# jimsnow/glome

Hardware: AMD Instinct MI355X
Metric: Mrays/sec + fps at 1920x1080 primary+shadow; 1/2/4/8 MI355X (higher is better)
Workload: dtype f32; 1 GPU; S3: 100,352-triangle heightfield under bih (BASELINE configs[2]), 1 light, primary + shadow rays, maxdepth 1; width=1920, height=1080, sampling=renderTile, 1 primary ray/pixel, launches_in_flight=4, frames_per_launch=32, transport=none (one GPU), frame_product=packed 0x00RRGGBB framebuffer (trace + blitTile fused, 4 B/pixel), bih_build=device (glome_sb_bih_dev / glome_sb_mesh_dev) for lists of 4096+ objects, device_bytes=14337692

## Files before the change

glome_amd/csrc/cull_kernels.hpp:

```cpp
#pragma once
#include <hip/hip_runtime.h>

#include "kernel_launch.hpp"
#include "rt_device.hpp"
#include "tiles.hpp"

constexpr int kCullThreads = 1024;
constexpr int kCullWaves = kCullThreads / 64, kCullPerWave = (int)kQueueChunk / kCullWaves;
static_assert(kCullWaves * kCullPerWave == (int)kQueueChunk && kQueueChunk == 64, "a chunk's live mask is one 64-bit word, a lane per position");

__device__ __forceinline__ bool queue_position(const DRenderArgs& A, uint32_t w, uint32_t& frame, uint32_t& item) {
  if (A.chunks_per_frame) {
    const uint32_t g = w / kQueueChunk, nf = (uint32_t)A.nframes;
    if (g >= A.chunks_per_frame * nf) return false;
    const uint32_t q = g / nf;
    frame = g - q * nf;
    w = q * kQueueChunk + (w % kQueueChunk);
    if (w >= A.total_waves) return false;
  } else {
    if (w >= A.total_waves * (uint32_t)A.nframes) return false;
    frame = w / A.total_waves;
    w -= frame * A.total_waves;
  }
  item = w;
  return true;
}

__device__ __forceinline__ bool item_live(const DScene& S, const Ray& r, bool valid) {
  for (uint32_t e = 0; e < S.n_entries; e++) {
    U4 ent = ldu4(S.entries, e);
    ent.x = uni(ent.x); ent.z = uni(ent.z);
    if (ent.z & RF_NOVIS) continue;
    U4 rec = ldu4(S.recs, ent.x);
    rec.x = uni(rec.x); rec.y = uni(rec.y);
    if ((rec.x & RF_KINDMASK) != R_BIH) return true;
    const F4 h0 = ld4u(S.bihhdr, 3 * rec.y), h1 = ld4u(S.bihhdr, 3 * rec.y + 1);
    if (uni(as_u(h0.w)) & BREF_LEAF) return true;
    float nearv, farv;
    bih_root_interval(r, h0, h1, kInf, nearv, farv);
    bih_clip_root_at_origin(nearv);
    if (wave_ballot(bih_root_enters(valid, nearv, farv)) != 0) return true;
  }
  return false;
}

__global__ void __launch_bounds__(kCullThreads) k_cull_items(DRenderArgs, uint32_t* list, uint32_t* masks, uint32_t nchunks) {
  const DRenderArgs& A = kernel_args<DRenderArgs>();
  __shared__ uint32_t s_bits[2], s_last, s_wave[kCullWaves], s_lo[kCullThreads], s_hi[kCullThreads], s_off[kCullThreads];
  const uint32_t tid = threadIdx.x, lane = tid & 63u, wave = tid >> 6, g = blockIdx.x;
  if (tid < 2) s_bits[tid] = 0;
  __syncthreads();
  uint32_t dead_px = 0;
  for (uint32_t k = 0; k < (uint32_t)kCullPerWave; k++) {
    const uint32_t j = wave * kCullPerWave + k;
    uint32_t frame, item;
    if (!queue_position(A, g * kQueueChunk + j, frame, item)) continue;
    const DItem it = ld_item_u(A.items, item);
    int px = 0, py = 0;
    size_t dense_off = 0;
    const bool valid = item_pixel(it, A.tiles, (int)lane, px, py, dense_off);
    const float xc = ldf(A.xc_tab, valid ? (uint32_t)px : 0u), yc = ldf(A.yc_tab, valid ? (uint32_t)py : 0u);
    const Ray ray = primary_ray(frame == 0 ? A.cam : A.more_cams[frame - 1], xc, yc);
    if (item_live(A.S, ray, valid)) {
      if (lane == 0) atomicOr(&s_bits[j >> 5], 1u << (j & 31u));
    } else {
      dead_px += (uint32_t)__builtin_popcountll(wave_ballot(valid));
      float depth = kInf;
      asm volatile("" : "+v"(depth));
      if (valid) store_pixel(A, frame, px, py, dense_off, ca(0, 0, 0, 0), depth);
    }
  }
  if (A.want_counters && dead_px && lane == 0) atomicAdd(&A.counters->rays_primary, (unsigned long long)dead_px);
  __syncthreads();
  if (tid == 0) {
    __hip_atomic_store(&masks[2 * g], s_bits[0], __ATOMIC_RELAXED, __HIP_MEMORY_SCOPE_AGENT);
    __hip_atomic_store(&masks[2 * g + 1], s_bits[1], __ATOMIC_RELAXED, __HIP_MEMORY_SCOPE_AGENT);
    asm volatile("s_waitcnt vmcnt(0)" ::: "memory");
    s_last = atomicAdd(&A.counters->cull_done, 1u) == nchunks - 1u ? 1u : 0u;
  }
  __syncthreads();
  if (!s_last) return;

  uint32_t running = 0;
  for (uint32_t base = 0; base < nchunks; base += kCullThreads) {
    const uint32_t c = base + tid;
    uint32_t lo = 0, hi = 0;
    if (c < nchunks) {
      lo = __hip_atomic_load(&masks[2 * c], __ATOMIC_RELAXED, __HIP_MEMORY_SCOPE_AGENT);
      hi = __hip_atomic_load(&masks[2 * c + 1], __ATOMIC_RELAXED, __HIP_MEMORY_SCOPE_AGENT);
    }
    const uint32_t cnt = (uint32_t)__builtin_popcount(lo) + (uint32_t)__builtin_popcount(hi);
    uint32_t incl = cnt;
    for (int o = 1; o < 64; o <<= 1) { const uint32_t v = __shfl_up(incl, o, 64); if ((int)lane >= o) incl += v; }
    if (lane == 63) s_wave[wave] = incl;
    __syncthreads();
    uint32_t before = 0, total = 0;
    for (uint32_t w = 0; w < (uint32_t)kCullWaves; w++) { const uint32_t v = s_wave[w]; total += v; if (w < wave) before += v; }
    s_lo[tid] = lo; s_hi[tid] = hi; s_off[tid] = running + before + incl - cnt;
    __syncthreads();
    for (uint32_t k = 0; k < 64; k++) {
      const uint32_t i = wave * 64 + k, ck = base + i;
      if (ck >= nchunks) break;
      const unsigned long long m = (unsigned long long)s_lo[i] | ((unsigned long long)s_hi[i] << 32);
      if (m == 0) continue;
      if ((m >> lane) & 1ull) {
        uint32_t frame = 0, item = 0;
        (void)queue_position(A, ck * kQueueChunk + lane, frame, item);
        list[s_off[i] + (uint32_t)__builtin_popcountll(m & ((1ull << lane) - 1ull))] = (frame << kListFrameShift) | item;
      }
    }
    running += total;
    __syncthreads();
  }
  if (tid == 0) {
    __hip_atomic_store(&A.counters->list_len, running, __ATOMIC_RELAXED, __HIP_MEMORY_SCOPE_AGENT);
    __hip_atomic_store(&A.counters->cull_done, 0u, __ATOMIC_RELAXED, __HIP_MEMORY_SCOPE_AGENT);
  }
}
```

glome_amd/csrc/runtime.hip:

```cpp
#include <hip/hip_runtime.h>

#include <cmath>
#include <cstdio>
#include <cstring>
#include <map>
#include <set>
#include <mutex>
#include <string>
#include <type_traits>
#include <vector>

#include "../../include/glome_hip.h"
#include "capi_shared.hpp"
#include "flatten.hpp"
#include "tiles.hpp"
#include "rt_device.hpp"
#include "instances.hpp"
#include "kernel_launch.hpp"
#include "bih_build_device.hpp"
#include "cull_kernels.hpp"
#include "mesh_update_kernels.hpp"
#include "bih_update_kernels.hpp"
#include "item_bih_update_kernels.hpp"
#include "sphere_bih_update_kernels.hpp"
// ... 422 lines not shown
    for (auto& b : boxes) bb = box_join(bb, b);
    if (bb.lo.x == -kInfinity || bb.lo.y == -kInfinity || bb.lo.z == -kInfinity || bb.hi.x == kInfinity || bb.hi.y == kInfinity || bb.hi.z == kInfinity)
      throw scene_error("bih: infinite bounding box");
    HIPCHK(ctx, hipSetDevice(ctx->device));
    auto T = std::make_shared<BihTree>();
    std::string err;
    if (!bihdev::build(boxes, v, bb, *T, ctx->stream, err, gpu_ms)) { ctx->err = sb->err = err; return GLOME_E_LIMIT; }
    T->order = v;
    Node nd; nd.kind = K_BIH; nd.bih = T;
    return G.add(nd);
  } catch (const scene_error& e) { ctx->err = sb->err = e.what(); return GLOME_E_SCENE; }
  catch (const std::exception& e) { ctx->err = sb->err = e.what(); return GLOME_E_INVALID; }
}

int32_t glome_sb_mesh_dev(glome_ctx* ctx, glome_sb* sb, const double* verts, int nv, const double* norms, int nn, const int32_t* tris, int nt, const int32_t* mats, int nm,
                          float* gpu_ms) {
  if (!ctx || !sb) { g_global_error = "null ctx or builder"; return GLOME_E_INVALID; }
  if (gpu_ms) *gpu_ms = 0;
  try {
    if (nv < 0 || nn < 0 || nt < 0 || nm < 0 || (nv && !verts) || (nn && !norms) || (nt && !tris) || (nm && !mats)) throw std::invalid_argument("bad mesh arrays");
    Graph& G = sb->graph;
    std::vector<D3> V, N;
    for (int k = 0; k < nv; k++) V.push_back(D3{verts[3 * k], verts[3 * k + 1], verts[3 * k + 2]});
    for (int k = 0; k < nn; k++) N.push_back(D3{norms[3 * k], norms[3 * k + 1], norms[3 * k + 2]});
    std::vector<MeshTri> T;
    for (int k = 0; k < nt; k++) { const int32_t* t = tris + 8 * k; T.push_back(MeshTri{t[0], t[1], t[2], t[3], t[4], t[5], t[6], t[7]}); }
    std::vector<int> M(mats, mats + nm);
    if (nt < 3) return G.mesh(std::move(V), std::move(N), std::move(T), std::move(M));
    std::vector<Box3> tbb;
    auto D = G.mesh_data(std::move(V), std::move(N), std::move(T), std::move(M), tbb);
    HIPCHK(ctx, hipSetDevice(ctx->device));
    std::string err;
    if (!bihdev::build_mesh(tbb, *D, ctx->stream, err, gpu_ms)) { ctx->err = sb->err = err; return GLOME_E_LIMIT; }
    return G.mesh_node(D);
  } catch (const scene_error& e) { ctx->err = sb->err = e.what(); return GLOME_E_SCENE; }
  catch (const std::exception& e) { ctx->err = sb->err = e.what(); return GLOME_E_INVALID; }
}

glome_scene* glome_scene_commit(glome_ctx* ctx, glome_sb* sb, int32_t root) {
  if (!ctx || !sb) { g_global_error = "null ctx or builder"; return nullptr; }
  FlatScene F;
  try {
    Flattener fl(sb_graph(sb), F);
    fl.run(root);
  } catch (std::exception& e) { ctx->err = e.what(); return nullptr; }
  (void)hipSetDevice(ctx->device);
  glome_scene* s = new glome_scene();
  s->ctx = ctx;
  int rc = 0;
  DScene& D = s->dev;
  rc |= upload(s, F.recs, &D.recs);
  rc |= upload(s, F.spheres, &D.spheres); rc |= upload(s, F.tris, &D.tris); rc |= upload(s, F.tripairs, &D.tripairs); rc |= upload(s, F.trinorms, &D.trinorms);
  rc |= upload(s, F.boxes, &D.boxes); rc |= upload(s, F.planes, &D.planes); rc |= upload(s, F.discs, &D.discs);
  rc |= upload(s, F.quadrics, &D.quadrics); rc |= upload(s, F.xfms, &D.xfms);
  rc |= upload(s, F.bihhdr, &D.bihhdr); rc |= upload(s, F.bihnodes, &D.bihnodes); rc |= upload(s, F.pknodes, &D.pknodes); D.pknodes_bytes = (uint32_t)(F.pknodes.size() * sizeof(F4));
  rc |= upload(s, F.meshhdr, &D.meshhdr); rc |= upload(s, F.meshnodes, &D.meshnodes); rc |= upload(s, F.mtris, &D.mtris);
  rc |= upload(s, F.mtrimeta, &D.mtrimeta); rc |= upload(s, F.mats, &D.mats); rc |= upload(s, F.wlights, &D.wlights); rc |= upload(s, F.matkids, &D.matkids);
  rc |= upload(s, F.entries, &D.entries);
  if (rc) { glome_scene_release(s); return nullptr; }
  D.n_entries = F.tier == 0 ? (uint32_t)F.entries.size() : 0;
  D.root_rec = F.root_rec; D.tier = F.tier; D.n_mats = (uint32_t)sb_graph(sb).mats.size(); D.tex_bits = F.tex_bits;
  const CommitRules R = commit_rules(sb_graph(sb), F);
  D.pk_generic_cap = R.caps.pk_generic_cap;
  if (getenv("GLOME_DEBUG_NO_GENERIC_PACKETS")) D.pk_generic_cap = 0;
  glome_scene_info& I = s->info;
  I.tier = (int32_t)F.tier; I.nesting_depth = F.nesting_depth;
  I.n_records = (int64_t)F.recs.size(); I.n_bih_nodes = (int64_t)F.bihnodes.size(); I.n_mesh_nodes = (int64_t)F.meshnodes.size() / 4;
  I.n_triangles = (int64_t)(F.tris.size() + F.mtris.size()) / 3; I.n_spheres = (int64_t)F.spheres.size();
  I.n_other_prims = F.n_other_prims; I.n_xfms = (int64_t)F.xfms.size() / 6; I.n_materials = D.n_mats;
  I.max_bih_depth = F.max_bih_depth; I.max_mesh_depth = F.max_mesh_depth;
  s->tr = R.traits;
  s->ovf_cap = R.caps.ovf_cap;
  for (MeshUpdateInfo& U : F.mesh_updates) {
    glome_scene::MeshUpd& m = s->meshes[U.node];
    if (upload(s, U.rows, &m.d_rows) || (!U.level_nodes.empty() && upload(s, U.level_nodes, &m.d_levels))) { glome_scene_release(s); return nullptr; }
    U.rows = {}; U.level_nodes = {};
    m.info = std::move(U);
  }
  for (LeafBihUpdateInfo& U : F.leaf_bih_updates) {
    glome_scene::LeafBihUpd& m = s->leaf_bihs[U.node];
    if ((!U.rows.empty() && upload(s, U.rows, &m.d_rows)) || (!U.level_nodes.empty() && (upload(s, U.level_nodes, &m.d_levels) || upload(s, U.level_off, &m.d_level_off)))) { glome_scene_release(s); return nullptr; }
    U.rows = {}; U.level_nodes = {};
    m.info = std::move(U);
  }
  for (InstBihInfo& B : F.inst_bihs) {
    glome_scene::InstBih& m = s->ibihs[B.node];
    if ((!B.level_nodes.empty() && upload(s, B.level_nodes, &m.d_levels)) || upload(s, B.rec_off, &m.d_rec_off) || upload(s, B.child_bound, &m.d_bounds)) { glome_scene_release(s); return nullptr; }
    B.level_nodes = {};
    m.info = std::move(B);
  }
  for (InstanceUpdateInfo& U : F.inst_updates) { const int node = U.node; s->insts[node] = std::move(U); }
  auto live_row = [&](int node, const double* b6) { s->live_slot[node] = (uint32_t)(s->live_bound0.size() / 6); s->live_bound0.insert(s->live_bound0.end(), b6, b6 + 6); };
  for (auto& m : s->meshes) live_row(m.first, m.second.info.bound6);
  for (auto& m : s->leaf_bihs) live_row(m.first, m.second.info.bound6);
  for (auto& m : s->ibihs) live_row(m.first, m.second.info.bound6);
  return s;
}
void glome_scene_release(glome_scene* s) {
  if (!s) return;
  (void)hipSetDevice(s->ctx->device);
  for (void* p : s->allocs) (void)hipFree(p);
  for (auto& st : s->inst_stage) { if (st.h) (void)hipHostFree(st.h); if (st.ev) (void)hipEventDestroy(st.ev); }
  if (s->d_inst_rows) (void)hipFree(s->d_inst_rows);
  delete s;
}
int glome_scene_get_info(const glome_scene* s, glome_scene_info* out) {
  if (!s || !out) return GLOME_E_INVALID;
  *out = s->info;
  return 0;
}

static bool other_slots_busy(glome_ctx* ctx) {
  for (int k = 0; k < glome_ctx::kSlots; k++) {
    const glome_ctx::Slot& sl = ctx->slots[k];
    if (k == ctx->cur || !sl.launched_on || sl.launched_on == ctx->stream) continue;
    if (hipStreamQuery(sl.launched_on) == hipErrorNotReady) return true;
  }
  (void)hipGetLastError();
  return false;
}
static int persistent_grid(glome_ctx* ctx, size_t lds_per_block, uint32_t total_work, int max_per_cu = 32, int min_per_cu = 0) {
  int cus = ctx->prop.multiProcessorCount;
  int per_cu = max_per_cu;
  if (lds_per_block) per_cu = std::min<int>(per_cu, (int)(160 * 1024 / lds_per_block));
  per_cu = std::max(per_cu, 1);
  if (ctx->grid_per_cu > 0) per_cu = std::min(per_cu, ctx->grid_per_cu);
  else if (min_per_cu > 0) {
    const bool alone = !other_slots_busy(ctx);
    const long per_wave = alone ? 16L : 64L;
    if (alone && min_per_cu >= 8) min_per_cu = 12;
    long want = ((long)total_work + per_wave * cus - 1) / (per_wave * cus);
    per_cu = (int)std::min<long>(per_cu, std::max<long>(min_per_cu, want));
  }
  long g = (long)cus * per_cu;
  return (int)std::max<long>(1, std::min<long>(g, total_work));
}
static int grid_floor(const glome_scene* s) { return s->tr.n_bih_nodes + s->tr.n_mesh_nodes < 4096 ? 3 : 8; }
static int ensure_overflow(glome_ctx* ctx, int grid, int waves_per_block, int ovf_cap) {
  size_t need = (size_t)grid * waves_per_block * (ovf_cap + 1) * 3 * 64 * sizeof(uint32_t);
  glome_ctx::Slot& sl = ctx->slot();
  if (need <= sl.ovf_bytes) return 0;
  if (sl.d_ovf) { HIPCHK(ctx, hipStreamSynchronize(ctx->stream)); HIPCHK(ctx, hipFree(sl.d_ovf)); sl.d_ovf = nullptr; sl.ovf_bytes = 0; }
  HIPCHK(ctx, hipMalloc((void**)&sl.d_ovf, need));
  sl.ovf_bytes = need;
  return 0;
}
static int ensure_scratch(glome_ctx* ctx, size_t need) {
  glome_ctx::Slot& sl = ctx->slot();
  if (need <= sl.scratch_bytes) return 0;
  if (sl.d_scratch) { HIPCHK(ctx, hipStreamSynchronize(ctx->stream)); HIPCHK(ctx, hipFree(sl.d_scratch)); sl.d_scratch = nullptr; sl.scratch_bytes = 0; }
  HIPCHK(ctx, hipMalloc((void**)&sl.d_scratch, need));
  sl.scratch_bytes = need;
  return 0;
}
static size_t list_chunks(size_t items) { return (items + kQueueChunk - 1) / kQueueChunk + kMaxBatchFrames; }
static int ensure_list(glome_ctx* ctx, uint32_t per_frame) {
  glome_ctx::Slot& sl = ctx->slot();
  const size_t need = (size_t)per_frame * kMaxBatchFrames;
  if (need <= sl.list_items) return 0;
  if (sl.d_list) { HIPCHK(ctx, hipStreamSynchronize(ctx->stream)); HIPCHK(ctx, hipFree(sl.d_list)); sl.d_list = nullptr; sl.list_items = 0; }
  HIPCHK(ctx, hipMalloc((void**)&sl.d_list, (need + 2 * list_chunks(need)) * sizeof(uint32_t)));
  sl.list_items = need;
  return 0;
}
static int device_error_status(glome_ctx* ctx, unsigned int e) {
  if (e & kErrNonUnit) {
    ctx->err = "a ray direction is not unit length: set glome_trace_params.faithful to trace such rays (the reference's own traversal)";
    return GLOME_E_INVALID;
  }
  if (e & kErrBadVertex) {
    ctx->err = "a mesh update met a vertex coordinate that is not finite: the scene's mesh is unspecified until a valid update"
               " (or a bih update, glome_scene_bih_update: then the bih is; or an Instance update, glome_scene_instance_update, met a matrix"
               " entry that is not finite or a bih item box that reaches infinity: then those Instances and the bih that holds them are; or a"
               " refit, glome_scene_bih_refit, met an item box or joined box that reaches infinity: then that bih and the bihs above it are;"
               " or a sphere bih update, glome_scene_sphere_bih_update, met a value that is not finite or a radius that is not positive: then"
               " that bih is); or an indexed bih update, glome_scene_bih_update_indexed_dev, met a vertex index outside [0, nv), read vertex 0 in"
               " its place, and left that bih unspecified";
    return GLOME_E_INVALID;
  }
  ctx->err = "device-side limit hit (traversal stack or CSG advance cap)";
  return GLOME_E_LIMIT;
}
static int poll_device_error(glome_ctx* ctx, glome_ctx::Slot& sl) {
  unsigned int e = 0;
  unsigned int* d = &sl.d_counters->error;
  HIPCHK(ctx, hipMemcpy(&e, d, sizeof(e), hipMemcpyDeviceToHost));
  if (!e) return 0;
  HIPCHK(ctx, hipMemset(d, 0, sizeof(e)));
  return device_error_status(ctx, e);
}
static int check_device_error(glome_ctx* ctx) { return poll_device_error(ctx, ctx->slot()); }

static int reset_counters(glome_ctx* ctx) {
  HIPCHK(ctx, hipMemsetAsync(ctx->slot().d_counters, 0, offsetof(DCounters, error), ctx->stream));
  return 0;
}

static bool launch_events(glome_ctx* ctx, hipEvent_t& e0, hipEvent_t& e1) {
  const bool pooled = ctx->timing && (ctx->timing_seen++ % ctx->timing_stride) == 0 && ctx->pool_used + 2 <= (int)ctx->pool.size();
  e0 = pooled ? ctx->pool[ctx->pool_used] : ctx->ev0; e1 = pooled ? ctx->pool[ctx->pool_used + 1] : ctx->ev1;
  if (pooled) ctx->pool_used += 2;
  return pooled;
}
static int launch_chosen(glome_scene* s, const Choice& ch, InstanceKind kind, int grid, size_t lds, const DRenderArgs& A) {
  glome_ctx* ctx = s->ctx;
  hipStream_t st = ctx->stream;
  if (ch.generic) {
    if (kind == KIND_SAMPLER) { if (ch.generic_counts) launch_ss_generic(grid, st, A); else launch_ss_generic_lean(grid, st, A); }
    else { if (ch.generic_counts) launch_render_generic(grid, st, A); else launch_render_generic_lean(grid, st, A); }
  } else {
    const FlatLaunch L{grid, lds, st, s->tr.stack_cap, ctx->slot().d_ovf, s->ovf_cap};
    if (kind == KIND_SAMPLER) { if (!launch_ss_flat(ch.key, L, A)) { ctx->err = "no sampler kernel instance for this scene class (build error)"; return GLOME_E_INVALID; } }
    else if (!launch_render_flat(ch.key, L, A)) { ctx->err = "no kernel instance for this scene class (build error)"; return GLOME_E_INVALID; }
  }
  HIPCHK(ctx, hipGetLastError());
  return 0;
}

static int render_impl(glome_scene* s, const glome_camera* cam, const glome_light* lights, int nlights, const glome_render_params* P,
                       float* rgbad_dev, uint32_t* packed_dev, glome_stats* stats, int dense, int nframes = 1, int64_t frame_stride = 0) {
  if (!s) return GLOME_E_INVALID;
  glome_ctx* ctx = s->ctx;
  if (!cam || (!rgbad_dev && !(dense != 1 && packed_dev)) || nlights < 0 || (nlights > 0 && !lights)) { ctx->err = "bad argument"; return GLOME_E_INVALID; }
  if (nlights > kMaxLights) { ctx->err = "too many lights"; return GLOME_E_LIMIT; }
  int rc = check_params(ctx, P);
  if (rc) return rc;
  if (P->mode != GLOME_MODE_TILE && P->mode != GLOME_MODE_SUBSAMPLE) { ctx->err = "unknown render mode"; return GLOME_E_INVALID; }
  if (P->mode == GLOME_MODE_SUBSAMPLE && P->blocksize > 65) { ctx->err = "GLOME_MODE_SUBSAMPLE supports tiles up to 65x65"; return GLOME_E_LIMIT; }
  HIPCHK(ctx, hipSetDevice(ctx->device));
  glome_ctx::TileTable* tt;
  const bool whole = P->mode == GLOME_MODE_TILE && dense == 0 && P->tile_first == 0 && P->tile_stride == 1;
  if ((rc = get_tiles(ctx, P, P->tile_first, P->tile_stride, &tt, whole ? 64 : 0))) return rc;
  DRenderArgs A;
  memset(&A, 0, sizeof(A));
  A.S = s->dev;
  memcpy(&A.cam, cam, sizeof(DCamera));
  if (nframes < 1 || nframes > kMaxBatchFrames) { ctx->err = "a launch carries 1..32 frames"; return GLOME_E_LIMIT; }
  if (nframes > 1 && (frame_stride <= 0 || frame_stride > 0xffffffffll)) { ctx->err = "frame batches: positive frame stride"; return GLOME_E_INVALID; }
  for (int f = 1; f < nframes; f++) memcpy(&A.more_cams[f - 1], cam + f, sizeof(DCamera));
  A.nframes = nframes; A.frame_stride = nframes > 1 ? (uint32_t)frame_stride : 0u;
  for (int i = 0; i < nlights; i++) {
    memcpy(A.lights[i].pos, lights[i].pos, 12); memcpy(A.lights[i].color, lights[i].color, 12);
    A.lights[i].rad = lights[i].rad; A.lights[i].shadow = lights[i].shadow;
  }
  A.nlights = nlights; A.width = P->width; A.height = P->height; A.fog = P->fog; A.maxdepth = P->maxdepth;
  memcpy(A.thresholds, P->thresholds, 16);
  A.tiles = tt->dev; A.tile_lut = tt->lut; A.items = tt->items; A.ntiles = (int)tt->host.size(); A.total_waves = tt->total_waves;
  {
    float* ct = nullptr;
    if ((rc = get_coord_tables(ctx, P->width, P->height, &ct))) return rc;
    A.xc_tab = ct; A.yc_tab = ct + P->width;
  }
  {
    A.chunks_per_frame = (nframes > 1 && P->mode == GLOME_MODE_TILE) ? (A.total_waves + kQueueChunk - 1) / kQueueChunk : 0u;
    const uint32_t tickets = A.chunks_per_frame ? A.chunks_per_frame * kQueueChunk * (uint32_t)nframes : A.total_waves * (uint32_t)nframes, round = kQueueChunk * kQueueShards;
    A.shard_cap = ((tickets + round - 1) / round) * kQueueChunk;
  }
  A.out5 = dense == 2 ? nullptr : rgbad_dev; A.packed = dense == 1 ? nullptr : packed_dev; A.counters = ctx->slot().d_counters; A.dense = dense != 0;
  const bool bare = !stats && P->mode == GLOME_MODE_TILE && !P->faithful && !P->count_work;
  if (!bare && (rc = reset_counters(ctx))) return rc;
  A.want_counters = (bare || (P->mode == GLOME_MODE_SUBSAMPLE && !stats)) ? 0 : 1;
  hipEvent_t ev_start = ctx->ev0, ev_stop = ctx->ev1;
  if (A.ntiles > 0 && P->mode == GLOME_MODE_SUBSAMPLE) {
    size_t npx = (size_t)tt->pixels;
    const size_t ctl_words = (size_t)(kSSHeads + 1) * kSSHeadStride + (size_t)A.ntiles * nframes * 8;
    if ((rc = ensure_scratch(ctx, npx * 5 * nframes * sizeof(float) + ctl_words * sizeof(unsigned int)))) return rc;
    A.scratch = ctx->slot().d_scratch;
    A.ss_cnt = (unsigned int*)(A.scratch + npx * 5 * nframes);
    A.ss_done = A.ss_cnt + (size_t)(kSSHeads + 1) * kSSHeadStride;
    A.ss_plane = (uint32_t)npx;
    A.blocksize = P->blocksize;
    for (int pass = 1; pass <= 5; pass++) {
      int rw, rh;
      ss_region_shape(pass, nframes >= 8 ? 2 : (nframes >= 3 ? 1 : 0), rw, rh);
      if (s->dev.tier != 0) { rw = (nframes >= 3 && pass >= 3) ? 2 : 1; rh = 1; }
      if (s->dev.tier != 0 && nframes >= 12) { static const int8_t W[6] = {0, 1, 2, 2, 2, 3}, H[6] = {0, 1, 1, 2, 2, 3}; rw = W[pass]; rh = H[pass]; }
      A.ss_rw[pass] = (int8_t)rw; A.ss_rh[pass] = (int8_t)rh;
    }
    HIPCHK(ctx, hipMemsetAsync(A.ss_cnt, 0, ctl_words * sizeof(unsigned int), ctx->stream));
    launch_events(ctx, ev_start, ev_stop);
    HIPCHK(ctx, hipEventRecord(ev_start, ctx->stream));
    const Choice ch = choose_sampler(s->tr, P->faithful != 0, P->count_work != 0, P->maxdepth, P->tile_stride);
    const size_t lds = ch.generic ? 0 : flat_lds_bytes(s->tr.stack_cap, ch.two_rows);
    const uint32_t items = ss_plan(A).first[6] * kSSHeads;
    int tgrid = persistent_grid(ctx, lds, (uint32_t)std::min<uint64_t>((uint64_t)items * 16, 0x7fffffffu), waves_per_cu(ch), grid_floor(s));
    tgrid = (int)std::min<uint32_t>((uint32_t)tgrid, items);
    if (!ch.generic && (rc = ensure_overflow(ctx, tgrid, 1, s->ovf_cap))) return rc;
    if ((rc = launch_chosen(s, ch, KIND_SAMPLER, tgrid, lds, A))) return rc;
    HIPCHK(ctx, hipEventRecord(ev_stop, ctx->stream));
  } else if (A.ntiles > 0) {
    const uint32_t items = A.total_waves * (uint32_t)nframes;
    const Choice ch = choose_render(s->tr, P->faithful != 0, P->count_work != 0, P->maxdepth, P->tile_stride, items);
    const size_t lds = ch.generic ? 0 : flat_lds_bytes(s->tr.stack_cap, ch.two_rows);
    const int grid = persistent_grid(ctx, lds, items, waves_per_cu(ch), grid_floor(s));
    if (!ch.generic && (rc = ensure_overflow(ctx, grid, 1, s->ovf_cap))) return rc;
    if (ch.two_rows) {
      if (A.total_waves > (1u << kListFrameShift)) { ctx->err = "frame too large"; return GLOME_E_INVALID; }
      if ((rc = ensure_list(ctx, A.total_waves))) return rc;
      A.list = ctx->slot().d_list;
    }
    const bool pooled = launch_events(ctx, ev_start, ev_stop), timed = stats || pooled;
    if (timed) HIPCHK(ctx, hipEventRecord(ev_start, ctx->stream));
    if (ch.two_rows) {
      const uint32_t nchunks = A.chunks_per_frame ? A.chunks_per_frame * (uint32_t)nframes : (items + kQueueChunk - 1) / kQueueChunk;
      glome_ctx::Slot& sl = ctx->slot();
      hipLaunchKernelGGL(k_cull_items, dim3(nchunks), dim3(kCullThreads), 0, ctx->stream, A, sl.d_list, sl.d_list + sl.list_items, nchunks);
      HIPCHK(ctx, hipGetLastError());
      sl.cull_total = items;
    }
    if ((rc = launch_chosen(s, ch, KIND_RENDER, grid, lds, A))) return rc;
    if (timed) HIPCHK(ctx, hipEventRecord(ev_stop, ctx->stream));
  }
  if (stats) {
    memset(stats, 0, sizeof(*stats));
    HIPCHK(ctx, hipStreamSynchronize(ctx->stream));
    DCounters c;
    HIPCHK(ctx, hipMemcpy(&c, ctx->slot().d_counters, sizeof(c), hipMemcpyDeviceToHost));
    stats->rays_primary = c.rays_primary; stats->rays_shadow = c.rays_shadow; stats->rays_secondary = c.rays_secondary;
    stats->bih_nodes = c.bih_nodes; stats->mesh_nodes = c.mesh_nodes; stats->prim_tests = c.prim_tests;
    if (A.ntiles > 0) HIPCHK(ctx, hipEventElapsedTime(&stats->kernel_ms, ev_start, ev_stop));
    stats->n_tiles = A.ntiles; stats->n_pixels = (int32_t)tt->pixels;
    ctx->slot().launched = false;
    if (c.error) {
      HIPCHK(ctx, hipMemset(&ctx->slot().d_counters->error, 0, sizeof(unsigned int)));
      return device_error_status(ctx, c.error);
    }
  } else if (A.ntiles > 0) { ctx->slot().launched = true; ctx->slot().launched_on = ctx->stream; }
  return 0;
}

int glome_render_dev(glome_scene* s, const glome_camera* cam, const glome_light* lights, int nlights, const glome_render_params* P,
                     float* rgbad_dev, uint32_t* packed_dev, glome_stats* stats) {
  return render_impl(s, cam, lights, nlights, P, rgbad_dev, packed_dev, stats, 0);
}
int glome_render_tiles_dev(glome_scene* s, const glome_camera* cam, const glome_light* lights, int nlights, const glome_render_params* P,
                           float* payload_dev, glome_stats* stats) {
  return render_impl(s, cam, lights, nlights, P, payload_dev, nullptr, stats, 1);
}
int glome_render_tiles_packed_dev(glome_scene* s, const glome_camera* cam, const glome_light* lights, int nlights, const glome_render_params* P,
                                  uint32_t* payload_dev, glome_stats* stats) {
  return render_impl(s, cam, lights, nlights, P, nullptr, payload_dev, stats, 2);
}

int glome_render_tiles_packed_batch_dev(glome_scene* s, const glome_camera* cams, int nframes, const glome_light* lights, int nlights,
                                        const glome_render_params* P, uint32_t* payload_dev, int64_t frame_stride_pixels, glome_stats* stats) {
  return render_impl(s, cams, lights, nlights, P, nullptr, payload_dev, stats, 2, nframes, frame_stride_pixels);
}
int glome_render_packed_batch_dev(glome_scene* s, const glome_camera* cams, int nframes, const glome_light* lights, int nlights,
                                  const glome_render_params* P, uint32_t* packed_dev, int64_t frame_stride_pixels, glome_stats* stats) {
  return render_impl(s, cams, lights, nlights, P, nullptr, packed_dev, stats, 0, nframes, frame_stride_pixels);
}

int glome_render(glome_scene* s, const glome_camera* cam, const glome_light* lights, int nlights, const glome_render_params* P, float* rgbad,
                 uint32_t* packed, glome_stats* stats) {
  if (!s) return GLOME_E_INVALID;
  glome_ctx* ctx = s->ctx;
  int rc = check_params(ctx, P);
  if (rc) return rc;
  if (!rgbad) { ctx->err = "null framebuffer"; return GLOME_E_INVALID; }
  HIPCHK(ctx, hipSetDevice(ctx->device));
  size_t np = (size_t)P->width * P->height;
  float* d5 = nullptr; uint32_t* dp = nullptr;
  HIPCHK(ctx, hipMalloc((void**)&d5, np * 5 * sizeof(float)));
  hipError_t e = hipMemcpy(d5, rgbad, np * 5 * sizeof(float), hipMemcpyHostToDevice);
  if (e == hipSuccess && packed) { e = hipMalloc((void**)&dp, np * 4); if (e == hipSuccess) e = hipMemcpy(dp, packed, np * 4, hipMemcpyHostToDevice); }
  if (e != hipSuccess) { ctx->err = hipGetErrorString(e); (void)hipFree(d5); if (dp) (void)hipFree(dp); return GLOME_E_HIP; }
  glome_stats local;
  rc = glome_render_dev(s, cam, lights, nlights, P, d5, dp, stats ? stats : &local);
  if (rc == 0) {
    e = hipMemcpy(rgbad, d5, np * 5 * sizeof(float), hipMemcpyDeviceToHost);
    if (e == hipSuccess && packed) e = hipMemcpy(packed, dp, np * 4, hipMemcpyDeviceToHost);
    if (e != hipSuccess) { ctx->err = hipGetErrorString(e); rc = GLOME_E_HIP; }
  }
  (void)hipFree(d5);
  if (dp) (void)hipFree(dp);
  return rc;
}

static int batch_grid(glome_ctx* ctx, size_t n, size_t lds) {
  size_t blocks = (n + 63) / 64;
  return (int)std::max<size_t>(1, std::min<size_t>(blocks, (size_t)persistent_grid(ctx, lds, 0x7fffffff) * 4));
}
static int flat_batch_launch(glome_scene* s, size_t n, FlatLaunch& L) {
  glome_ctx* ctx = s->ctx;
  const size_t lds = flat_lds_bytes(s->tr.stack_cap);
  const int grid = batch_grid(ctx, n, lds);
  if (int rc = ensure_overflow(ctx, grid, 1, s->ovf_cap)) return rc;
  L = FlatLaunch{grid, lds, ctx->stream, s->tr.stack_cap, ctx->slot().d_ovf, s->ovf_cap};
  return 0;
}
int glome_rayint_batch_dev(glome_scene* s, size_t n, const float* ox, const float* oy, const float* oz, const float* dx, const float* dy,
                           const float* dz, const float* tmax, float* t, int32_t* prim, float* nx, float* ny, float* nz, int32_t* tex8) {
  if (!s) return GLOME_E_INVALID;
  glome_ctx* ctx = s->ctx;
  if (n == 0) return 0;
  if (!ox || !oy || !oz || !dx || !dy || !dz || !tmax) { ctx->err = "null ray stream"; return GLOME_E_INVALID; }
  HIPCHK(ctx, hipSetDevice(ctx->device));
  RayStream R{ox, oy, oz, dx, dy, dz, tmax};
  HitStream H{t, prim, nx, ny, nz, tex8};
  if (s->dev.tier == 0) {
    FlatLaunch L;
    if (int rc = flat_batch_launch(s, n, L)) return rc;
    launch_rayint_batch_flat(L, s->dev, n, R, H, ctx->slot().d_counters);
  } else {
    if (int rc = reset_counters(ctx)) return rc;
    launch_rayint_batch_generic(batch_grid(ctx, n, 0), ctx->stream, s->dev, n, R, H, ctx->slot().d_counters);
  }
  ctx->slot().launched = true; ctx->slot().launched_on = ctx->stream;
  HIPCHK(ctx, hipGetLastError());
  return 0;
}
int glome_shadow_batch_dev(glome_scene* s, size_t n, const float* ox, const float* oy, const float* oz, const float* dx, const float* dy,
                           const float* dz, const float* tmax, uint8_t* occluded) {
  if (!s) return GLOME_E_INVALID;
  glome_ctx* ctx = s->ctx;
  if (n == 0) return 0;
  if (!ox || !oy || !oz || !dx || !dy || !dz || !tmax || !occluded) { ctx->err = "null stream"; return GLOME_E_INVALID; }
  HIPCHK(ctx, hipSetDevice(ctx->device));
  RayStream R{ox, oy, oz, dx, dy, dz, tmax};
  if (s->dev.tier == 0) {
    FlatLaunch L;
    if (int rc = flat_batch_launch(s, n, L)) return rc;
    launch_shadow_batch_flat(L, s->dev, n, R, occluded, ctx->slot().d_counters);
  } else {
    if (int rc = reset_counters(ctx)) return rc;
    launch_shadow_batch_generic(batch_grid(ctx, n, 0), ctx->stream, s->dev, n, R, occluded, ctx->slot().d_counters);
  }
  ctx->slot().launched = true; ctx->slot().launched_on = ctx->stream;
  HIPCHK(ctx, hipGetLastError());
  return 0;
}

struct Staging {
  glome_ctx* ctx;
  std::vector<void*> bufs;
  ~Staging() { for (void* p : bufs) (void)hipFree(p); }
  template <class T> T* in(const T* h, size_t n) {
    T* d = nullptr;
    if (hipMalloc((void**)&d, std::max<size_t>(1, n) * sizeof(T)) != hipSuccess) return nullptr;
    bufs.push_back(d);
    if (h && hipMemcpy(d, h, n * sizeof(T), hipMemcpyHostToDevice) != hipSuccess) return nullptr;
    return d;
  }
  int rays(const float* const (&h)[7], size_t n, float* (&d)[7]) {
    for (int k = 0; k < 7; k++) if (!(d[k] = in(h[k], n))) { ctx->err = "staging allocation failed"; return GLOME_E_HIP; }
    return 0;
  }
};
int glome_rayint_batch(glome_scene* s, size_t n, const float* ox, const float* oy, const float* oz, const float* dx, const float* dy,
                       const float* dz, const float* tmax, float* t, int32_t* prim, float* nx, float* ny, float* nz, int32_t* tex8) {
  if (!s) return GLOME_E_INVALID;
  glome_ctx* ctx = s->ctx;
  if (n == 0) return 0;
  if (!ox || !oy || !oz || !dx || !dy || !dz || !tmax) { ctx->err = "null ray stream"; return GLOME_E_INVALID; }
  HIPCHK(ctx, hipSetDevice(ctx->device));
  Staging st{ctx, {}};
  float* din[7];
  if (int rc = st.rays({ox, oy, oz, dx, dy, dz, tmax}, n, din)) return rc;
  float* dt = t ? st.in<float>(nullptr, n) : nullptr;
  int32_t* dprim = prim ? st.in<int32_t>(nullptr, n) : nullptr;
  float* dnx = nx ? st.in<float>(nullptr, n) : nullptr;
  float* dny = ny ? st.in<float>(nullptr, n) : nullptr;
  float* dnz = nz ? st.in<float>(nullptr, n) : nullptr;
  int32_t* dtex = tex8 ? st.in<int32_t>(nullptr, 8 * n) : nullptr;
  int rc = glome_rayint_batch_dev(s, n, din[0], din[1], din[2], din[3], din[4], din[5], din[6], dt, dprim, dnx, dny, dnz, dtex);
  if (rc) return rc;
  HIPCHK(ctx, hipStreamSynchronize(ctx->stream));
  if ((rc = check_device_error(ctx))) return rc;
  if (t) HIPCHK(ctx, hipMemcpy(t, dt, n * 4, hipMemcpyDeviceToHost));
  if (prim) HIPCHK(ctx, hipMemcpy(prim, dprim, n * 4, hipMemcpyDeviceToHost));
  if (nx) HIPCHK(ctx, hipMemcpy(nx, dnx, n * 4, hipMemcpyDeviceToHost));
  if (ny) HIPCHK(ctx, hipMemcpy(ny, dny, n * 4, hipMemcpyDeviceToHost));
  if (nz) HIPCHK(ctx, hipMemcpy(nz, dnz, n * 4, hipMemcpyDeviceToHost));
  if (tex8) HIPCHK(ctx, hipMemcpy(tex8, dtex, n * 32, hipMemcpyDeviceToHost));
  return 0;
}
int glome_shadow_batch(glome_scene* s, size_t n, const float* ox, const float* oy, const float* oz, const float* dx, const float* dy,
                       const float* dz, const float* tmax, uint8_t* occluded) {
  if (!s) return GLOME_E_INVALID;
  glome_ctx* ctx = s->ctx;
  if (n == 0) return 0;
  if (!ox || !oy || !oz || !dx || !dy || !dz || !tmax || !occluded) { ctx->err = "null stream"; return GLOME_E_INVALID; }
  HIPCHK(ctx, hipSetDevice(ctx->device));
  Staging st{ctx, {}};
  float* din[7];
  if (int rc = st.rays({ox, oy, oz, dx, dy, dz, tmax}, n, din)) return rc;
  uint8_t* docc = st.in<uint8_t>(nullptr, n);
  int rc = glome_shadow_batch_dev(s, n, din[0], din[1], din[2], din[3], din[4], din[5], din[6], docc);
  if (rc) return rc;
  HIPCHK(ctx, hipStreamSynchronize(ctx->stream));
  if ((rc = check_device_error(ctx))) return rc;
  HIPCHK(ctx, hipMemcpy(occluded, docc, n, hipMemcpyDeviceToHost));
  return 0;
}
int glome_inside_batch(glome_scene* s, size_t n, const float* px, const float* py, const float* pz, uint8_t* inside) {
  if (!s) return GLOME_E_INVALID;
  glome_ctx* ctx = s->ctx;
  if (n == 0) return 0;
  if (!px || !py || !pz || !inside) { ctx->err = "null stream"; return GLOME_E_INVALID; }
  HIPCHK(ctx, hipSetDevice(ctx->device));
  Staging st{ctx, {}};
  float *dx = st.in(px, n), *dy = st.in(py, n), *dz = st.in(pz, n);
  uint8_t* din = st.in<uint8_t>(nullptr, n);
  if (!dx || !dy || !dz || !din) { ctx->err = "staging allocation failed"; return GLOME_E_HIP; }
  if (int rcc = reset_counters(ctx)) return rcc;
  launch_inside_batch(batch_grid(ctx, n, 0), ctx->stream, s->dev, n, dx, dy, dz, din, ctx->slot().d_counters);
  HIPCHK(ctx, hipGetLastError());
  HIPCHK(ctx, hipStreamSynchronize(ctx->stream));
  int rc = check_device_error(ctx);
  if (rc) return rc;
  HIPCHK(ctx, hipMemcpy(inside, din, n, hipMemcpyDeviceToHost));
  return 0;
}

static int quiesce(glome_ctx* ctx) {
  HIPCHK(ctx, hipStreamSynchronize(ctx->stream));
  for (auto& sl : ctx->slots)
    if (sl.launched_on && sl.launched_on != ctx->stream) (void)hipStreamSynchronize(sl.launched_on);
  (void)hipGetLastError();
  return 0;
}
template <class Dev> static int run_blocking(glome_ctx* ctx, float* gpu_ms, Dev dev) {
  if (gpu_ms) HIPCHK(ctx, hipEventRecord(ctx->ev0, ctx->stream));
  if (int rc = dev()) return rc;
  if (gpu_ms) HIPCHK(ctx, hipEventRecord(ctx->ev1, ctx->stream));
  HIPCHK(ctx, hipStreamSynchronize(ctx->stream));
  if (gpu_ms) HIPCHK(ctx, hipEventElapsedTime(gpu_ms, ctx->ev0, ctx->ev1));
  return check_device_error(ctx);
}
struct StageIn {
  Staging stg;
  bool ok = true;
  template <class T> T* operator()(const T* h, size_t n) { T* d = stg.in<T>(h, n); ok = ok && d; return d; }
};
template <class Check, class Validate, class Stage> static int blocking_update(glome_scene* s, float* gpu_ms, Check check, Validate validate, Stage stage, bool empty = false) {
  if (!s) return GLOME_E_INVALID;
  glome_ctx* ctx = s->ctx;
  if (gpu_ms) *gpu_ms = 0;
  if (int rc = check()) return rc;
  if (int rc = validate()) return rc;
  if (empty) return 0;
  HIPCHK(ctx, hipSetDevice(ctx->device));
  if (int rc = quiesce(ctx)) return rc;
  StageIn in{{ctx, {}}};
  auto dev = stage(in);
  if (!in.ok) { ctx->err = "staging allocation failed"; return GLOME_E_HIP; }
  return run_blocking(ctx, gpu_ms, dev);
}
struct UpdateSpan {
  glome_ctx* ctx;
  bool split;
  hipEvent_t e0 = nullptr, e1 = nullptr;
  UpdateSpan(glome_ctx* c, const char* split_env) : ctx(c), split(split_env && getenv(split_env) != nullptr) {}
  hipError_t begin() { return ctx->timing && launch_events(ctx, e0, e1) ? hipEventRecord(e0, ctx->stream) : (e1 = nullptr, hipSuccess); }
  hipError_t end() { return e1 ? hipEventRecord(e1, ctx->stream) : hipSuccess; }
  hipError_t stage() {
    if (!split) return hipSuccess;
    const hipError_t e = end();
    return e != hipSuccess ? e : begin();
  }
};
template <class K, class... Args> static void launch_lanes(glome_ctx* ctx, K kernel, uint32_t n, Args... args) {
  if (!n) return;
  const uint32_t max_items = (uint32_t)ctx->prop.multiProcessorCount * 32u * 4u;
  hipLaunchKernelGGL(kernel, dim3(std::min<uint32_t>((n + 63u) >> 6, max_items)), dim3(64), 0, ctx->stream, args...);
}
static void mark_launched(glome_ctx* ctx) { ctx->slot().launched = true; ctx->slot().launched_on = ctx->stream; }
static int ensure_ws(glome_scene* s, float4*& d_ws, size_t words) {
  if (d_ws) return 0;
  void* d = nullptr;
  HIPCHK(s->ctx, hipMalloc(&d, words * sizeof(float4)));
  s->allocs.push_back(d);
  d_ws = (float4*)d;
  return 0;
}
static int accepted(glome_scene* s, const char* what, const UpdateAnswer& plain, const NestedAnswer& nested) {
  const UpdateAnswer& A = s->nested_on ? nested : plain;
  if (!A.ok) { s->ctx->err = std::string(what) + " refused: " + A.why_not; return GLOME_E_INVALID; }
  return 0;
}
template <class T> static upd::IndexedPts<T> indexed_pts(glome_ctx* ctx, const void* verts_dev, int nv, const int32_t* idx_dev) {
  return upd::IndexedPts<T>{(const T*)verts_dev, idx_dev, (uint32_t)nv, &ctx->slot().d_counters->error};
}
template <class Src> constexpr bool kSphereSrc = std::is_same<Src, sphupd::SphPacked64>::value || std::is_same<Src, sphupd::SphSplit32>::value;
template <class Src> static void launch_bound32(glome_ctx* ctx, Src src, uint32_t n, float4* part, float start, float4* hdr) {
  const uint32_t blocks = std::max<uint32_t>(1u, std::min<uint32_t>((n + upd::kBoundBlock - 1) / upd::kBoundBlock, (uint32_t)upd::kBoundMaxBlocks));
  if constexpr (kSphereSrc<Src>) {
    hipLaunchKernelGGL(sphupd::k_sph_bound<Src>, dim3(blocks), dim3(upd::kBoundBlock), 0, ctx->stream, src, n, part);
  } else {
    upd::DBoundArgs<Src> A;
    A.src = src; A.nv = n; A.part = part; A.error = &ctx->slot().d_counters->error;
    hipLaunchKernelGGL(upd::k_points_bound<Src>, dim3(blocks), dim3(upd::kBoundBlock), 0, ctx->stream, A);
  }
  hipLaunchKernelGGL(upd::k_bound_store, dim3(1), dim3(64), 0, ctx->stream, (const float4*)part, blocks, start, hdr);
}
static void launch_levels(glome_ctx* ctx, const bihupd::DLevelArgs& A, const std::vector<uint32_t>& level_off, const uint32_t* merged_off) {
  const size_t levels = level_off.empty() ? 0 : level_off.size() - 1;
  auto width = [&](size_t l) { return level_off[l + 1] - level_off[l]; };
  for (size_t l = 0; l < levels;) {
    size_t e = l;
    while (merged_off && e < levels && width(e) <= (uint32_t)bihupd::kMergeBlock) e++;
    if (e > l + 1) {
      hipLaunchKernelGGL(bihupd::k_bih_levels_merged, dim3(1), dim3(bihupd::kMergeBlock), 0, ctx->stream, A, merged_off, (uint32_t)l, (uint32_t)e);
      l = e;
    } else {
      launch_lanes(ctx, bihupd::k_bih_level, width(l), A, level_off[l], width(l));
// ... 1138 lines not shown
```

Baseline: 31350 Mrays/s.

## Probe one lane per item before full-wave cull test; shrink cull blocks

The cull kernel now has wave 0 test a single probe pixel per item across all 64 positions at once, marking items proven live without a full per-pixel test. Only unproven items get the full 64-lane root test, distributed round-robin across waves, with live bits merged via one atomic per wave. Block size drops to 512 threads, and the last-block compaction scan handles two chunks per thread using register readlanes instead of shared arrays. It also rejects multi-frame launches that are not chunk-interleaved.

```diff
diff --git a/glome_amd/csrc/cull_kernels.hpp b/glome_amd/csrc/cull_kernels.hpp
--- a/glome_amd/csrc/cull_kernels.hpp
+++ b/glome_amd/csrc/cull_kernels.hpp
@@ -5,28 +5,32 @@
 #include "rt_device.hpp"
 #include "tiles.hpp"
 
-constexpr int kCullThreads = 1024;
-constexpr int kCullWaves = kCullThreads / 64, kCullPerWave = (int)kQueueChunk / kCullWaves;
-static_assert(kCullWaves * kCullPerWave == (int)kQueueChunk && kQueueChunk == 64, "a chunk's live mask is one 64-bit word, a lane per position");
+constexpr int kCullThreads = 512;
+constexpr int kCullWaves = kCullThreads / 64;
+constexpr int kCullProbeLane = 36;
+constexpr int kScanChunks = 1024, kScanPerThread = kScanChunks / kCullThreads, kScanPerWave = kScanChunks / kCullWaves;
+static_assert(kCullThreads % 64 == 0 && kScanPerThread * kCullThreads == kScanChunks && kQueueChunk == 64, "a chunk's live mask is one 64-bit word, a lane per position");
 
-__device__ __forceinline__ bool queue_position(const DRenderArgs& A, uint32_t w, uint32_t& frame, uint32_t& item) {
+__device__ __forceinline__ void chunk_position(const DRenderArgs& A, uint32_t g, uint32_t& frame, uint32_t& first) {
+  frame = 0;
   if (A.chunks_per_frame) {
-    const uint32_t g = w / kQueueChunk, nf = (uint32_t)A.nframes;
-    if (g >= A.chunks_per_frame * nf) return false;
-    const uint32_t q = g / nf;
+    const uint32_t nf = (uint32_t)A.nframes, q = g / nf;
     frame = g - q * nf;
-    w = q * kQueueChunk + (w % kQueueChunk);
-    if (w >= A.total_waves) return false;
-  } else {
-    if (w >= A.total_waves * (uint32_t)A.nframes) return false;
-    frame = w / A.total_waves;
-    w -= frame * A.total_waves;
+    g = q;
   }
-  item = w;
-  return true;
+  first = g * kQueueChunk;
 }
 
-__device__ __forceinline__ bool item_live(const DScene& S, const Ray& r, bool valid) {
+__device__ __forceinline__ DItem ld_item(const DItem* p, uint32_t i) {
+#if defined(__HIP_DEVICE_COMPILE__)
+  return as_global(p)[i];
+#else
+  return p[i];
+#endif
+}
+
+__device__ __forceinline__ bool lane_enters(const DScene& S, const Ray& r, bool valid) {
+  bool in = false;
   for (uint32_t e = 0; e < S.n_entries; e++) {
     U4 ent = ldu4(S.entries, e);
     ent.x = uni(ent.x); ent.z = uni(ent.z);
@@ -39,36 +43,61 @@
     float nearv, farv;
     bih_root_interval(r, h0, h1, kInf, nearv, farv);
     bih_clip_root_at_origin(nearv);
-    if (wave_ballot(bih_root_enters(valid, nearv, farv)) != 0) return true;
+    in = in || bih_root_enters(valid, nearv, farv);
   }
-  return false;
+  return in;
 }
+__device__ __forceinline__ bool item_live(const DScene& S, const Ray& r, bool valid) { return wave_ballot(lane_enters(S, r, valid)) != 0; }
 
 __global__ void __launch_bounds__(kCullThreads) k_cull_items(DRenderArgs, uint32_t* list, uint32_t* masks, uint32_t nchunks) {
   const DRenderArgs& A = kernel_args<DRenderArgs>();
-  __shared__ uint32_t s_bits[2], s_last, s_wave[kCullWaves], s_lo[kCullThreads], s_hi[kCullThreads], s_off[kCullThreads];
-  const uint32_t tid = threadIdx.x, lane = tid & 63u, wave = tid >> 6, g = blockIdx.x;
-  if (tid < 2) s_bits[tid] = 0;
+  __shared__ uint32_t s_bits[2], s_todo[2], s_last, s_wave[kCullWaves];
+  const uint32_t tid = threadIdx.x, lane = tid & 63u, wave = uni(tid >> 6), g = blockIdx.x;
+  uint32_t frame, first;
+  chunk_position(A, g, frame, first);
+  const uint32_t npos = min((uint32_t)kQueueChunk, A.total_waves - first);
+  const DCamera cam = frame == 0 ? A.cam : A.more_cams[frame - 1];
+
+  if (wave == 0) {
+    const bool pos = lane < npos;
+    const DItem it = ld_item(A.items, first + (pos ? lane : 0u));
+    int px = 0, py = 0;
+    size_t dense_off = 0;
+    if (!item_pixel(it, A.tiles, kCullProbeLane, px, py, dense_off)) (void)item_pixel(it, A.tiles, 0, px, py, dense_off);
+    const Ray ray = primary_ray(cam, ldf(A.xc_tab, (uint32_t)px), ldf(A.yc_tab, (uint32_t)py));
+    const LaneMask proven = wave_ballot(pos && lane_enters(A.S, ray, pos));
+    const LaneMask todo = wave_ballot(pos) & ~proven;
+    if (lane == 0) {
+      s_bits[0] = (uint32_t)proven; s_bits[1] = (uint32_t)(proven >> 32);
+      s_todo[0] = (uint32_t)todo; s_todo[1] = (uint32_t)(todo >> 32);
+    }
+  }
   __syncthreads();
+
+  const LaneMask todo = (LaneMask)uni(s_todo[0]) | ((LaneMask)uni(s_todo[1]) << 32);
+  LaneMask mine = wave_ballot(((todo >> lane) & 1ull) != 0 && (uint32_t)__builtin_popcountll(todo & ((1ull << lane) - 1ull)) % (uint32_t)kCullWaves == wave);
+  LaneMask found = 0;
   uint32_t dead_px = 0;
-  for (uint32_t k = 0; k < (uint32_t)kCullPerWave; k++) {
-    const uint32_t j = wave * kCullPerWave + k;
-    uint32_t frame, item;
-    if (!queue_position(A, g * kQueueChunk + j, frame, item)) continue;
-    const DItem it = ld_item_u(A.items, item);
+  for (; mine; mine &= mine - 1ull) {
+    const uint32_t j = (uint32_t)__builtin_ctzll(mine);
+    const DItem it = ld_item_u(A.items, first + j);
     int px = 0, py = 0;
     size_t dense_off = 0;
     const bool valid = item_pixel(it, A.tiles, (int)lane, px, py, dense_off);
     const float xc = ldf(A.xc_tab, valid ? (uint32_t)px : 0u), yc = ldf(A.yc_tab, valid ? (uint32_t)py : 0u);
-    const Ray ray = primary_ray(frame == 0 ? A.cam : A.more_cams[frame - 1], xc, yc);
+    const Ray ray = primary_ray(cam, xc, yc);
     if (item_live(A.S, ray, valid)) {
-      if (lane == 0) atomicOr(&s_bits[j >> 5], 1u << (j & 31u));
+      found |= 1ull << j;
     } else {
       dead_px += (uint32_t)__builtin_popcountll(wave_ballot(valid));
       float depth = kInf;
       asm volatile("" : "+v"(depth));
       if (valid) store_pixel(A, frame, px, py, dense_off, ca(0, 0, 0, 0), depth);
     }
+  }
+  if (found && lane == 0) {
+    if ((uint32_t)found) atomicOr(&s_bits[0], (uint32_t)found);
+    if ((uint32_t)(found >> 32)) atomicOr(&s_bits[1], (uint32_t)(found >> 32));
   }
   if (A.want_counters && dead_px && lane == 0) atomicAdd(&A.counters->rays_primary, (unsigned long long)dead_px);
   __syncthreads();
@@ -82,31 +111,41 @@
   if (!s_last) return;
 
   uint32_t running = 0;
-  for (uint32_t base = 0; base < nchunks; base += kCullThreads) {
-    const uint32_t c = base + tid;
-    uint32_t lo = 0, hi = 0;
-    if (c < nchunks) {
-      lo = __hip_atomic_load(&masks[2 * c], __ATOMIC_RELAXED, __HIP_MEMORY_SCOPE_AGENT);
-      hi = __hip_atomic_load(&masks[2 * c + 1], __ATOMIC_RELAXED, __HIP_MEMORY_SCOPE_AGENT);
+  for (uint32_t base = 0; base < nchunks; base += (uint32_t)kScanChunks) {
+    uint32_t lo[kScanPerThread], hi[kScanPerThread], cnt = 0;
+#pragma unroll
+    for (int p = 0; p < kScanPerThread; p++) {
+      const uint32_t c = base + tid * (uint32_t)kScanPerThread + (uint32_t)p;
+      lo[p] = 0; hi[p] = 0;
+      if (c < nchunks) {
+        lo[p] = __hip_atomic_load(&masks[2 * c], __ATOMIC_RELAXED, __HIP_MEMORY_SCOPE_AGENT);
+        hi[p] = __hip_atomic_load(&masks[2 * c + 1], __ATOMIC_RELAXED, __HIP_MEMORY_SCOPE_AGENT);
+      }
+      cnt += (uint32_t)__builtin_popcount(lo[p]) + (uint32_t)__builtin_popcount(hi[p]);
     }
-    const uint32_t cnt = (uint32_t)__builtin_popcount(lo) + (uint32_t)__builtin_popcount(hi);
     uint32_t incl = cnt;
     for (int o = 1; o < 64; o <<= 1) { const uint32_t v = __shfl_up(incl, o, 64); if ((int)lane >= o) incl += v; }
     if (lane == 63) s_wave[wave] = incl;
     __syncthreads();
     uint32_t before = 0, total = 0;
     for (uint32_t w = 0; w < (uint32_t)kCullWaves; w++) { const uint32_t v = s_wave[w]; total += v; if (w < wave) before += v; }
-    s_lo[tid] = lo; s_hi[tid] = hi; s_off[tid] = running + before + incl - cnt;
-    __syncthreads();
-    for (uint32_t k = 0; k < 64; k++) {
-      const uint32_t i = wave * 64 + k, ck = base + i;
-      if (ck >= nchunks) break;
-      const unsigned long long m = (unsigned long long)s_lo[i] | ((unsigned long long)s_hi[i] << 32);
-      if (m == 0) continue;
-      if ((m >> lane) & 1ull) {
-        uint32_t frame = 0, item = 0;
-        (void)queue_position(A, ck * kQueueChunk + lane, frame, item);
-        list[s_off[i] + (uint32_t)__builtin_popcountll(m & ((1ull << lane) - 1ull))] = (frame << kListFrameShift) | item;
+    uint32_t off[kScanPerThread];
+    off[0] = running + before + incl - cnt;
+#pragma unroll
+    for (int p = 1; p < kScanPerThread; p++) off[p] = off[p - 1] + (uint32_t)__builtin_popcount(lo[p - 1]) + (uint32_t)__builtin_popcount(hi[p - 1]);
+    uint32_t ck = base + wave * (uint32_t)kScanPerWave, cframe = 0, cfirst = 0;
+    if (ck < nchunks) chunk_position(A, ck, cframe, cfirst);
+    cframe = uni(cframe); cfirst = uni(cfirst);
+    for (uint32_t l = 0; l < 64u && ck < nchunks; l++) {
+#pragma unroll
+      for (int p = 0; p < kScanPerThread; p++, ck++) {
+        const unsigned long long m = (unsigned long long)(uint32_t)__builtin_amdgcn_readlane((int)lo[p], (int)l) | ((unsigned long long)(uint32_t)__builtin_amdgcn_readlane((int)hi[p], (int)l) << 32);
+        if (m != 0) {
+          const uint32_t o = (uint32_t)__builtin_amdgcn_readlane((int)off[p], (int)l);
+          if ((m >> lane) & 1ull) list[o + (uint32_t)__builtin_popcountll(m & ((1ull << lane) - 1ull))] = (cframe << kListFrameShift) | (cfirst + lane);
+        }
+        if (A.chunks_per_frame && ++cframe != (uint32_t)A.nframes) continue;
+        cframe = 0; cfirst += kQueueChunk;
       }
     }
     running += total;
diff --git a/glome_amd/csrc/runtime.hip b/glome_amd/csrc/runtime.hip
--- a/glome_amd/csrc/runtime.hip
+++ b/glome_amd/csrc/runtime.hip
@@ -748,6 +748,7 @@
     const bool pooled = launch_events(ctx, ev_start, ev_stop), timed = stats || pooled;
     if (timed) HIPCHK(ctx, hipEventRecord(ev_start, ctx->stream));
     if (ch.two_rows) {
+      if (nframes > 1 && !A.chunks_per_frame) { ctx->err = "a flagship launch of several frames is interleaved by chunks"; return GLOME_E_INVALID; }
       const uint32_t nchunks = A.chunks_per_frame ? A.chunks_per_frame * (uint32_t)nframes : (items + kQueueChunk - 1) / kQueueChunk;
       glome_ctx::Slot& sl = ctx->slot();
       hipLaunchKernelGGL(k_cull_items, dim3(nchunks), dim3(kCullThreads), 0, ctx->stream, A, sl.d_list, sl.d_list + sl.list_items, nchunks);
```

New measurement: 33100 Mrays/s (median of 6 runs). 1.06x the previous value.
